# JiapengWu/TeMP

Measured on AMD Instinct MI355X. Metric: edges/sec (fwd+bwd) RGCN+GRU seq_len=15, higher is better.
Workload: dtype f32

## Files before the change

### temp_amd/csrc/gru_chain_hx.hpp

```cpp
#pragma once
#include "hx_pack.hpp"

namespace temp {

#define CHX_STATE_SCALE 16384.f
#define CHX_STATE_INV (1.f / 16384.f)

#define CHX_STAMP_EVENTS 8
#define CHX_STAMP_BLOCK (2 * CH_MAX_STEPS * CHX_STAMP_EVENTS)
#define CHX_STAMP_WORDS (2 * 2 * CHX_STAMP_BLOCK)
template <int DEV>
__device__ __forceinline__ long long* chx_stamp_rows(long long* stamp, int kernel, int role, bool first_wave, int lane) {
  if constexpr (DEV) {
    if (!stamp || !first_wave || lane != 0) return nullptr;
    const int mid = (int)(gridDim.x >> 1);
    const int sel = blockIdx.x == 0 ? 0 : ((int)blockIdx.x == mid ? 1 : -1);
    return sel < 0 ? nullptr : stamp + ((size_t)(kernel * 2 + sel) * 2 + role) * (CH_MAX_STEPS * CHX_STAMP_EVENTS);
  }
  return nullptr;
}
#define CHX_STAMP(s, k) do { if constexpr (DEV) { if (stp) stp[(s) * CHX_STAMP_EVENTS + (k)] = (long long)__builtin_readcyclecounter(); } } while (0)

struct ChainGeomHx {
  int NT, NS;
  int NTb, NSb;
  int lda, ldz;
  int ldp, ldpa;
  int ldh;
};
__host__ __device__ inline ChainGeomHx chain_geom_hx(int D) {
  ChainGeomHx g;
  g.NT = (3 * D + 31) >> 5; g.NS = (D + 15) >> 4;
  g.NTb = (D + 31) >> 5; g.NSb = (((3 * D + 15) >> 4) + 7) & ~7;
  g.lda = g.NT * 32 + 4; g.ldz = g.NTb * 32 + 4;
  g.ldp = g.NS * 32 + 16; g.ldpa = g.NSb * 32 + 16;
  g.ldh = g.NS * 16 + 4;
  return g;
}
inline size_t chain_lds_fwd_hx(int D, int ms) {
  const ChainGeomHx g = chain_geom_hx(D);
  return (size_t)CH_SLOTS * g.lda * 4 + 2 * (size_t)CH_SLOTS * g.ldp + (size_t)CH_SLOTS * g.ldh * 4 + (size_t)g.NT * 32 * 4 + (2 * CH_SLOTS + 1) * (size_t)ms * 4;
}
inline size_t chain_lds_bwd_hx(int D, int ms) {
  const ChainGeomHx g = chain_geom_hx(D);
  return 2 * (size_t)CH_SLOTS * g.ldpa + 2 * (size_t)CH_SLOTS * g.ldz * 4 + (2 * CH_SLOTS + 3) * (size_t)ms * 4 + CH_SLOTS * 4 + 4 * (size_t)D * 4;
}
inline size_t chain_hx_fwd_items(int D) { const ChainGeomHx g = chain_geom_hx(D); return (size_t)g.NS * g.NT * 128; }
inline size_t chain_hx_bwd_items(int D) { const ChainGeomHx g = chain_geom_hx(D); return (size_t)g.NSb * g.NTb * 128; }
inline size_t chain_hx_pack_floats(int D) {
  const ChainGeomHx g = chain_geom_hx(D);
  return (chain_hx_fwd_items(D) + chain_hx_bwd_items(D)) * 4 + (size_t)(g.NT + g.NTb) * 32;
}

template <int VARIANT, int TPW, int MW, int NMW = 4, int TWOSETS = 0>
__global__ void __launch_bounds__(64 * (NMW + MW)) k_gru_chain_fwd_hx(ChainArgs a, const float* __restrict__ gi, float* __restrict__ H,
                                                                       float* __restrict__ saved) {
  extern __shared__ __attribute__((aligned(16))) float lds[];
  constexpr int PASSES = CH_SLOTS / MW;
  const int D = a.D, D4 = D >> 2;
  const int G = (VARIANT == TEMP_GRU_TORCH) ? 3 * D : D;
  const ChainGeomHx g = chain_geom_hx(D);
  const int NT = g.NT, NS = g.NS, lda = g.lda, ldp = g.ldp, ldh = g.ldh;
  float* accb = lds;
  char* hpl = (char*)(accb + CH_SLOTS * lda);
  float* hb = (float*)(hpl + 2 * CH_SLOTS * ldp);
  float* ivt = hb + CH_SLOTS * ldh;
  int* tabb = (int*)(ivt + NT * 32);
  float* decb = (float*)(tabb + CH_SLOTS * a.max_steps);
  int* flagb = (int*)(decb + CH_SLOTS * a.max_steps);
  const int tid = threadIdx.x, wave = __builtin_amdgcn_readfirstlane(tid >> 6), lane = tid & 63;
  const size_t plane = a.plane;

  for (int p = blockIdx.x; p < a.n_panels; p += gridDim.x) {
    const int rnn_id = a.panel[4 * p], s0 = a.panel[4 * p + 1], ns = a.panel[4 * p + 2];
    const ChainRnn R = a.rnn[rnn_id];
    for (int i = tid; i < 2 * CH_SLOTS * ldp / 16; i += blockDim.x) reinterpret_cast<hx_u32x4*>(hpl)[i] = hx_u32x4{0u, 0u, 0u, 0u};
    for (int i = tid; i < CH_SLOTS * ldh; i += blockDim.x) hb[i] = 0.f;
    for (int i = tid; i < NT * 32; i += blockDim.x) ivt[i] = hx_inv_scale(R.kf[i]) * CHX_STATE_INV;
    for (int i = tid; i < ns * CH_SLOTS; i += blockDim.x) {
      const int e = a.rows[(size_t)s0 * CH_SLOTS + i];
      tabb[i] = e;
      decb[i] = e >= 0 ? decay_factor(a.dt[e & CH_ROW_MASK], a.lambda, R.decay_wb) : 0.f;
    }
    if (tid < ns) flagb[tid] = a.sinfo[4 * (size_t)(s0 + tid)];
    __syncthreads();

    if (wave < NMW) {
      const int li = lane & 31, hh = lane >> 5;
      bool tval[TPW];
      int tidx[TPW];
#pragma unroll
      for (int j = 0; j < TPW; ++j) { tidx[j] = wave + NMW * j; tval[j] = tidx[j] < NT; if (!tval[j]) tidx[j] = NT - 1; }
      f32x16 acc[TPW];
#pragma unroll
      for (int j = 0; j < TPW; ++j)
#pragma unroll
        for (int r = 0; r < 16; ++r) acc[j][r] = 0.f;
      const hx_u32x4* wp = reinterpret_cast<const hx_u32x4*>(R.wf);
      constexpr bool ONESET = NMW > 4 && !TWOSETS;
      constexpr bool PREF = !(NMW > 4 && TWOSETS);
      hx_u32x4 w[ONESET ? 1 : 2][2][TPW] = {};
      auto wload = [&](hx_u32x4 (&wr)[TPW], int sl, int pl) {
#pragma unroll
        for (int j = 0; j < TPW; ++j)
          if (tval[j]) wr[j] = wp[((size_t)(sl * NT + tidx[j]) * 2 + pl) * 64 + lane];
      };
      const int rot = (a.dbg & 64) ? 0 : (int)(blockIdx.x >> 3) % NS;
      wload(w[0][0], rot, 0); wload(w[0][1], rot, 1);
      if constexpr (!ONESET) { wload(w[1][0], rot + 1 < NS ? rot + 1 : 0, 0); wload(w[1][1], rot + 1 < NS ? rot + 1 : 0, 1); }
      const char* hrow = hpl + (size_t)li * ldp + 16 * hh;
      const int pl1 = CH_SLOTS * ldp;
      for (int s = 0; s < ns; ++s) {
        const int flags = flagb[s];
        if ((flags & 1) && !(a.dbg & 1)) {
          hx_u32x4 FH = *reinterpret_cast<const hx_u32x4*>(hrow + 32 * rot), FL = *reinterpret_cast<const hx_u32x4*>(hrow + pl1 + 32 * rot), NH, NL;
          int sl_cur = rot;
          auto slab = [&](auto set_c, int sl1, int sl2) {
            constexpr int SET = decltype(set_c)::value;
            if constexpr (PREF) {
              NH = *reinterpret_cast<const hx_u32x4*>(hrow + 32 * sl1);
              NL = *reinterpret_cast<const hx_u32x4*>(hrow + pl1 + 32 * sl1);
            } else {
              FH = *reinterpret_cast<const hx_u32x4*>(hrow + 32 * sl_cur);
              FL = *reinterpret_cast<const hx_u32x4*>(hrow + pl1 + 32 * sl_cur);
              sl_cur = sl1;
            }
            const hx_f16x8 ah = hx_frag(FH), al = hx_frag(FL);
            __builtin_amdgcn_sched_barrier(0);
#pragma unroll
            for (int j = 0; j < TPW; ++j) acc[j] = __builtin_amdgcn_mfma_f32_32x32x16_f16(hx_frag(w[SET][1][j]), ah, acc[j], 0, 0, 0);
            __builtin_amdgcn_sched_barrier(0);
            wload(w[SET][1], sl2, 1);
            __builtin_amdgcn_sched_barrier(0);
#pragma unroll
            for (int j = 0; j < TPW; ++j) acc[j] = __builtin_amdgcn_mfma_f32_32x32x16_f16(hx_frag(w[SET][0][j]), al, acc[j], 0, 0, 0);
#pragma unroll
            for (int j = 0; j < TPW; ++j) acc[j] = __builtin_amdgcn_mfma_f32_32x32x16_f16(hx_frag(w[SET][0][j]), ah, acc[j], 0, 0, 0);
            __builtin_amdgcn_sched_barrier(0);
            wload(w[SET][0], sl2, 0);
            if constexpr (PREF) { FH = NH; FL = NL; }
          };
          auto at = [&](int j) { const int v = rot + j; return v < NS ? v : v - NS; };
          if constexpr (ONESET) {
            for (int j = 0; j < NS; ++j) slab(std::integral_constant<int, 0>(), at(j + 1 < NS ? j + 1 : 0), at(j + 1 < NS ? j + 1 : 0));
          } else {
          int j = 0;
          for (; j + 1 < NS; j += 2) {
            slab(std::integral_constant<int, 0>(), at(j + 1), at(j + 2 < NS ? j + 2 : 0));
            slab(std::integral_constant<int, 1>(), at(j + 2 < NS ? j + 2 : 0), at(j + 3 < NS ? j + 3 : 1));
          }
          if (j < NS) slab(std::integral_constant<int, 0>(), at(0), at(0));
          }
#pragma unroll
          for (int j = 0; j < TPW; ++j) {
            if (!tval[j]) continue;
            float* dst = accb + (size_t)li * lda + tidx[j] * 32 + 4 * hh;
#pragma unroll
            for (int qq = 0; qq < 4; ++qq) {
              st4(dst + 8 * qq, make_float4(acc[j][4 * qq], acc[j][4 * qq + 1], acc[j][4 * qq + 2], acc[j][4 * qq + 3]));
              acc[j][4 * qq] = 0.f; acc[j][4 * qq + 1] = 0.f; acc[j][4 * qq + 2] = 0.f; acc[j][4 * qq + 3] = 0.f;
            }
          }
        }
        __syncthreads();
        __syncthreads();
      }
    } else {
      const int mw = wave - NMW, c4 = lane, col = 4 * c4;
      const bool cact = c4 < D4;
      const int colc = cact ? col : 0;
      const float4 bhr = ld4(R.b_hh + colc), bhz = ld4(R.b_hh + D + colc), bhn = ld4(R.b_hh + 2 * D + colc);
      int erow[PASSES];
      float4 g0[PASSES], g1[PASSES], g2[PASSES];
      auto prefetch = [&](int s) {
#pragma unroll
        for (int ps = 0; ps < PASSES; ++ps) {
          const int e = tabb[s * CH_SLOTS + ps * MW + mw];
          erow[ps] = e;
          const bool ok = e >= 0 && cact && !(a.dbg & 4);
          const int er = e & CH_ROW_MASK;
          const float* src = gi + (ok ? (size_t)(a.gi_index ? a.gi_index[er] : er) * G + col : 0);
          if (VARIANT == TEMP_GRU_TORCH) { g0[ps] = ld4(src); g1[ps] = ld4(src + (ok ? D : 0)); g2[ps] = ld4(src + (ok ? 2 * D : 0)); }
          else { g0[ps] = zero4(); g1[ps] = zero4(); g2[ps] = ld4(src); }
        }
      };
      prefetch(0);
      for (int s = 0; s < ns; ++s) {
        const int flags = flagb[s];
        __syncthreads();
#pragma unroll
        for (int ps = 0; ps < PASSES; ++ps) {
          const int slot = ps * MW + mw;
          const int e = erow[ps];
          if (e < 0 || !cact) continue;
          const size_t row = (size_t)(e & CH_ROW_MASK);
          const bool hp = (e & CH_HAS_PREV) != 0;
          float4 ar = zero4(), az = zero4(), an = zero4(), hd = zero4();
          if (hp) {
            const float* ab = accb + (size_t)slot * lda + col;
            const float dec = decb[s * CH_SLOTS + slot];
            const float4 pr = ld4(ab), pz = ld4(ab + D), pn = ld4(ab + 2 * D);
            const float4 ivr = ld4(ivt + col), ivz = ld4(ivt + D + col), ivn = ld4(ivt + 2 * D + col);
            ar = make_float4(pr.x * (ivr.x * dec), pr.y * (ivr.y * dec), pr.z * (ivr.z * dec), pr.w * (ivr.w * dec));
            az = make_float4(pz.x * (ivz.x * dec), pz.y * (ivz.y * dec), pz.z * (ivz.z * dec), pz.w * (ivz.w * dec));
            an = make_float4(pn.x * (ivn.x * dec), pn.y * (ivn.y * dec), pn.z * (ivn.z * dec), pn.w * (ivn.w * dec));
            hd = scale4(ld4(hb + (size_t)slot * ldh + col), dec);
          }
          float o_h[4], o_r[4], o_z[4], o_n[4], o_hn[4];
          const float arv[4] = {ar.x, ar.y, ar.z, ar.w}, azv[4] = {az.x, az.y, az.z, az.w}, anv[4] = {an.x, an.y, an.z, an.w};
          const float hdv[4] = {hd.x, hd.y, hd.z, hd.w};
          const float g0v[4] = {g0[ps].x, g0[ps].y, g0[ps].z, g0[ps].w}, g1v[4] = {g1[ps].x, g1[ps].y, g1[ps].z, g1[ps].w};
          const float g2v[4] = {g2[ps].x, g2[ps].y, g2[ps].z, g2[ps].w};
          const float brv[4] = {bhr.x, bhr.y, bhr.z, bhr.w}, bzv[4] = {bhz.x, bhz.y, bhz.z, bhz.w}, bnv[4] = {bhn.x, bhn.y, bhn.z, bhn.w};
#pragma unroll
          for (int k = 0; k < 4; ++k) {
            float xr = arv[k], xz = azv[k];
            if (VARIANT == TEMP_GRU_TORCH) { xr += g0v[k]; xz += g1v[k]; }
            const float rg = gate_sigmoid(xr + brv[k]);
            const float zg = gate_sigmoid(xz + bzv[k]);
            const float hn = anv[k] + bnv[k];
            const float ng = gate_tanh(g2v[k] + rg * hn);
            o_h[k] = (VARIANT == TEMP_GRU_TORCH) ? ((1.f - zg) * ng + zg * hdv[k]) : (ng + zg * (hdv[k] - ng));
            o_r[k] = rg; o_z[k] = zg; o_n[k] = ng; o_hn[k] = hn;
          }
          const float4 h4 = make_float4(o_h[0], o_h[1], o_h[2], o_h[3]);
          st4(hb + (size_t)slot * ldh + col, h4);
          hx_u32x2 SH, SL;
          hx_split4(h4, CHX_STATE_SCALE, SH, SL);
          char* hdst = hpl + (size_t)slot * ldp + 2 * col;
          *reinterpret_cast<hx_u32x2*>(hdst) = SH;
          *reinterpret_cast<hx_u32x2*>(hdst + CH_SLOTS * ldp) = SL;
          const size_t o = row * D + col;
          if (a.dbg & 2) continue;
          if (flags & 2) st4(H + o, h4);
          st4(saved + o, make_float4(o_r[0], o_r[1], o_r[2], o_r[3]));
          st4(saved + plane + o, make_float4(o_z[0], o_z[1], o_z[2], o_z[3]));
          st4(saved + 2 * plane + o, make_float4(o_n[0], o_n[1], o_n[2], o_n[3]));
          st4(saved + 3 * plane + o, make_float4(o_hn[0], o_hn[1], o_hn[2], o_hn[3]));
          st4(saved + 4 * plane + o, hd);
        }
        __syncthreads();
        if (s + 1 < ns) prefetch(s + 1);
      }
    }
    __syncthreads();
  }
}

struct ChainX {
  const float* x;
  const int32_t* x_index;
  const float* b_ih[TEMP_CHAIN_MAX_RNN];
  const hx_u32x4* wi[TEMP_CHAIN_MAX_RNN];
};
inline size_t chain_lds_fwd_x(int D, int ms) {
  const ChainGeomHx g = chain_geom_hx(D);
  return (size_t)CH_SLOTS * (3 * D + 4) * 4 + 4 * (size_t)CH_SLOTS * g.ldp + (size_t)CH_SLOTS * (D + 4) * 4 + CH_SLOTS * 4 + (2 * CH_SLOTS + 1) * (size_t)ms * 4;
}
template <int TPW, int MW, int NMW, int DEV = 0>
__global__ void __launch_bounds__(64 * (NMW + MW)) k_gru_chain_fwd_x(ChainArgs a, ChainX X, float* __restrict__ H, float* __restrict__ saved) {
  extern __shared__ __attribute__((aligned(16))) float lds[];
  constexpr int PASSES = CH_SLOTS / MW;
  const int D = a.D, D4 = D >> 2, G3 = 3 * D;
  const ChainGeomHx g = chain_geom_hx(D);
  const int NT = g.NT, NS = g.NS, ldp = g.ldp;
  const int lda = G3 + 4, ldn = D + 4;
  float* accb = lds;
  char* hpl = (char*)(accb + CH_SLOTS * lda);
  char* xpl = hpl + 2 * CH_SLOTS * ldp;
  float* gin = (float*)(xpl + 2 * CH_SLOTS * ldp);
  unsigned* xkey = (unsigned*)(gin + CH_SLOTS * ldn);
  int* tabb = (int*)(xkey + CH_SLOTS);
  float* decb = (float*)(tabb + CH_SLOTS * a.max_steps);
  int* flagb = (int*)(decb + CH_SLOTS * a.max_steps);
  const int tid = threadIdx.x, wave = __builtin_amdgcn_readfirstlane(tid >> 6), lane = tid & 63;
  const size_t plane = a.plane;
  const int dbg = DEV ? a.dbg : 0;

  if (wave < NMW) {
  for (int p = blockIdx.x; p < a.n_panels; p += gridDim.x) {
    const int rnn_id = a.panel[4 * p], s0 = a.panel[4 * p + 1], ns = a.panel[4 * p + 2];
    const ChainRnn R = a.rnn[rnn_id];
    for (int i = tid; i < 4 * CH_SLOTS * ldp / 16; i += blockDim.x) reinterpret_cast<hx_u32x4*>(hpl)[i] = hx_u32x4{0u, 0u, 0u, 0u};
    for (int i = tid; i < ns * CH_SLOTS; i += blockDim.x) {
      const int e = a.rows[(size_t)s0 * CH_SLOTS + i];
      tabb[i] = e;
      decb[i] = e >= 0 ? decay_factor(a.dt[e & CH_ROW_MASK], a.lambda, R.decay_wb) : 0.f;
    }
    if (tid < ns) flagb[tid] = a.sinfo[4 * (size_t)(s0 + tid)];
    __syncthreads();

      const int li = lane & 31, hh = lane >> 5;
      bool tval[TPW];
      int tidx[TPW];
#pragma unroll
      for (int j = 0; j < TPW; ++j) { tidx[j] = wave + NMW * j; tval[j] = tidx[j] < NT; if (!tval[j]) tidx[j] = NT - 1; }
      f32x16 acc[TPW];
#pragma unroll
      for (int j = 0; j < TPW; ++j)
#pragma unroll
        for (int r = 0; r < 16; ++r) acc[j][r] = 0.f;
      const hx_u32x4* wph = reinterpret_cast<const hx_u32x4*>(R.wf);
      const hx_u32x4* wpi = X.wi[rnn_id];
      hx_u32x4 w[2][TPW] = {};
      const std::integral_constant<int, 0> P0;
      const std::integral_constant<int, 1> P1;
      auto wload = [&](const hx_u32x4* wp, int sl, auto pl_c, int ln) __attribute__((always_inline)) {
        constexpr int pl = decltype(pl_c)::value;
#pragma unroll
        for (int j = 0; j < TPW; ++j)
          if (tval[j]) w[pl][j] = *reinterpret_cast<const hx_u32x4*>(reinterpret_cast<const char*>(wp) + (unsigned)((((sl * NT + tidx[j]) * 2 + pl) * 64 + ln) * 16));
      };
      const int rot = (dbg & 64) ? 0 : (int)(blockIdx.x >> 3) % NS;
      auto at = [&](int j) { const int v = rot + j; return v < NS ? v : v - NS; };
      const bool prio = !(dbg & 4096);
      bool holds_ih = true;
      wload(wpi, rot, P0, lane); wload(wpi, rot, P1, lane);
      auto walk = [&](const bool prod, const char* pl0, const hx_u32x4* wcur, const hx_u32x4* wnext) __attribute__((always_inline)) {
        int ln = lane;
        asm volatile("" : "+v"(ln));
        const char* arow = pl0 + (size_t)(ln & 31) * ldp + 16 * (ln >> 5);
        const int pl1 = CH_SLOTS * ldp;
        hx_u32x4 FH = *reinterpret_cast<const hx_u32x4*>(arow + 32 * rot), FL = *reinterpret_cast<const hx_u32x4*>(arow + pl1 + 32 * rot), NH, NL;
        if (prio) __builtin_amdgcn_s_setprio(2);
        for (int j = 0; j < NS; ++j) {
          const bool last = j + 1 == NS;
          const int sn = at(last ? 0 : j + 1);
          const hx_u32x4* wn = last ? wnext : wcur;
          NH = *reinterpret_cast<const hx_u32x4*>(arow + 32 * sn);
          NL = *reinterpret_cast<const hx_u32x4*>(arow + pl1 + 32 * sn);
          const hx_f16x8 ah = hx_frag(FH), al = hx_frag(FL);
          __builtin_amdgcn_sched_barrier(0);
#pragma unroll
          for (int t = 0; t < TPW; ++t) {
            if (prod) acc[t] = __builtin_amdgcn_mfma_f32_32x32x16_f16(hx_frag(w[1][t]), ah, acc[t], 0, 0, 0);
            else asm volatile("" : : "v"(w[1][t]));
          }
          __builtin_amdgcn_sched_barrier(0);
          wload(wn, sn, P1, ln);
          __builtin_amdgcn_sched_barrier(0);
          if (prod) {
#pragma unroll
            for (int t = 0; t < TPW; ++t) acc[t] = __builtin_amdgcn_mfma_f32_32x32x16_f16(hx_frag(w[0][t]), al, acc[t], 0, 0, 0);
#pragma unroll
            for (int t = 0; t < TPW; ++t) acc[t] = __builtin_amdgcn_mfma_f32_32x32x16_f16(hx_frag(w[0][t]), ah, acc[t], 0, 0, 0);
          } else {
#pragma unroll
            for (int t = 0; t < TPW; ++t) asm volatile("" : : "v"(w[0][t]));
          }
          __builtin_amdgcn_sched_barrier(0);
          wload(wn, sn, P0, ln);
          FH = NH; FL = NL;
        }
        if (prio) __builtin_amdgcn_s_setprio(0);
      };
      auto xprod = [&]() __attribute__((always_inline)) {
        if (!holds_ih) { wload(wpi, rot, P0, lane); wload(wpi, rot, P1, lane); }
        walk(!(dbg & (1 | 2048)), xpl, wpi, wph);
        holds_ih = false;
        const float f = hx_inv_scale(xkey[li]) * CHX_STATE_SCALE;
#pragma unroll
        for (int j = 0; j < TPW; ++j)
#pragma unroll
          for (int r = 0; r < 16; ++r) acc[j][r] *= f;
      };
      long long* stp = p == (int)blockIdx.x ? chx_stamp_rows<DEV>(a.stamp, 0, 0, wave == 0, lane) : nullptr;
      if (ns > 0) {
        __syncthreads();
        xprod();
        __syncthreads();
      }
      for (int s = 0; s < ns; ++s) {
        const int flags = flagb[s];
        CHX_STAMP(s, 0);
#pragma unroll
        for (int j = 0; j < TPW; ++j) {
          if (!tval[j]) continue;
#pragma unroll
          for (int qq = 0; qq < 4; ++qq) {
            const int c = tidx[j] * 32 + 8 * qq + 4 * hh;
            if (c < 2 * D || c >= G3) continue;
            st4(gin + (size_t)li * ldn + (c - 2 * D), make_float4(acc[j][4 * qq], acc[j][4 * qq + 1], acc[j][4 * qq + 2], acc[j][4 * qq + 3]));
            acc[j][4 * qq] = 0.f; acc[j][4 * qq + 1] = 0.f; acc[j][4 * qq + 2] = 0.f; acc[j][4 * qq + 3] = 0.f;
          }
        }
        if ((flags & 1) && !(dbg & 1)) {
          if (holds_ih) { wload(wph, rot, P0, lane); wload(wph, rot, P1, lane); }
          walk(true, hpl, wph, wpi);
          holds_ih = true;
        }
        CHX_STAMP(s, 1);
#pragma unroll
        for (int j = 0; j < TPW; ++j) {
          if (!tval[j]) continue;
          float* dst = accb + (size_t)li * lda + tidx[j] * 32 + 4 * hh;
#pragma unroll
          for (int qq = 0; qq < 4; ++qq) {
            if (tidx[j] * 32 + 8 * qq + 4 * hh < G3) st4(dst + 8 * qq, make_float4(acc[j][4 * qq], acc[j][4 * qq + 1], acc[j][4 * qq + 2], acc[j][4 * qq + 3]));
            acc[j][4 * qq] = 0.f; acc[j][4 * qq + 1] = 0.f; acc[j][4 * qq + 2] = 0.f; acc[j][4 * qq + 3] = 0.f;
          }
        }
        CHX_STAMP(s, 2);
        __syncthreads();
        CHX_STAMP(s, 3);
        if (s + 1 < ns) xprod();
        CHX_STAMP(s, 4);
        __syncthreads();
        CHX_STAMP(s, 5);
      }
    __syncthreads();
  }
  } else {
  for (int p = blockIdx.x; p < a.n_panels; p += gridDim.x) {
    const int rnn_id = a.panel[4 * p], s0 = a.panel[4 * p + 1], ns = a.panel[4 * p + 2];
    const ChainRnn R = a.rnn[rnn_id];
    for (int i = tid; i < 4 * CH_SLOTS * ldp / 16; i += blockDim.x) reinterpret_cast<hx_u32x4*>(hpl)[i] = hx_u32x4{0u, 0u, 0u, 0u};
    for (int i = tid; i < ns * CH_SLOTS; i += blockDim.x) {
      const int e = a.rows[(size_t)s0 * CH_SLOTS + i];
      tabb[i] = e;
      decb[i] = e >= 0 ? decay_factor(a.dt[e & CH_ROW_MASK], a.lambda, R.decay_wb) : 0.f;
    }
    if (tid < ns) flagb[tid] = a.sinfo[4 * (size_t)(s0 + tid)];
    __syncthreads();

      const int mw = wave - NMW, c4 = lane, col = 4 * c4;
      const bool cact = c4 < D4;
      const int colc = cact ? col : 0;
      const float* bih = X.b_ih[rnn_id];
      const float4 br = add4(ld4(bih + colc), ld4(R.b_hh + colc)), bz = add4(ld4(bih + D + colc), ld4(R.b_hh + D + colc));
      const float4 bhn = ld4(R.b_hh + 2 * D + colc), bin = ld4(bih + 2 * D + colc);
      float4 ivr, ivz, ivn;
      {
        const hx_u32x4 kr = *reinterpret_cast<const hx_u32x4*>(R.kf + colc), kz = *reinterpret_cast<const hx_u32x4*>(R.kf + D + colc);
        const hx_u32x4 kn = *reinterpret_cast<const hx_u32x4*>(R.kf + 2 * D + colc);
        auto iv = [](const hx_u32x4 k) { return make_float4(hx_inv_scale(k[0]) * CHX_STATE_INV, hx_inv_scale(k[1]) * CHX_STATE_INV,
                                                            hx_inv_scale(k[2]) * CHX_STATE_INV, hx_inv_scale(k[3]) * CHX_STATE_INV); };
        ivr = iv(kr); ivz = iv(kz); ivn = iv(kn);
      }
      float4 hdr[PASSES];
      float4 xr[PASSES];
      int xi[PASSES];
#pragma unroll
      for (int ps = 0; ps < PASSES; ++ps) hdr[ps] = zero4();
      typedef const int32_t __attribute__((address_space(4))) * chx_const_idx;
      const chx_const_idx xidx = (chx_const_idx)(uintptr_t)X.x_index;
      auto xindex = [&](int s) __attribute__((always_inline)) {
        int e[PASSES];
#pragma unroll
        for (int ps = 0; ps < PASSES; ++ps) e[ps] = tabb[s * CH_SLOTS + ps * MW + mw];
        __builtin_amdgcn_sched_barrier(0);
#pragma unroll
        for (int ps = 0; ps < PASSES; ++ps) {
          const int es = __builtin_amdgcn_readfirstlane(e[ps]);
          xi[ps] = (es >= 0 && !(dbg & 4)) ? xidx[es & CH_ROW_MASK] : -1;
        }
      };
      auto xload = [&]() __attribute__((always_inline)) {
#pragma unroll
        for (int ps = 0; ps < PASSES; ++ps) {
          xr[ps] = zero4();
          if (xi[ps] >= 0 && cact) xr[ps] = ld4(X.x + (size_t)xi[ps] * D + col);
        }
      };
      auto xsplit = [&]() __attribute__((always_inline)) {
#pragma unroll
        for (int ps = 0; ps < PASSES; ++ps) {
          const int slot = ps * MW + mw;
          const unsigned key = hx_wave_max(cact ? hx_abs_bits4(xr[ps]) : 0u);
          if (cact) {
            hx_u32x2 SH, SL;
            hx_split4(xr[ps], hx_scale(key), SH, SL);
            char* xd = xpl + (size_t)slot * ldp + 2 * col;
            *reinterpret_cast<hx_u32x2*>(xd) = SH;
            *reinterpret_cast<hx_u32x2*>(xd + CH_SLOTS * ldp) = SL;
          }
          if (lane == 0) xkey[slot] = key;
        }
      };
      long long* stp = p == (int)blockIdx.x ? chx_stamp_rows<DEV>(a.stamp, 0, 1, mw == 0, lane) : nullptr;
      if (ns > 0) {
        xindex(0);
        xload();
        if (ns > 1) xindex(1);
        xsplit();
        __syncthreads();
        if (ns > 1) xload();
        __syncthreads();
      }
      for (int s = 0; s < ns; ++s) {
        const int flags = flagb[s];
        CHX_STAMP(s, 0);
        if (s + 2 < ns) xindex(s + 2);
        if (s + 1 < ns) xsplit();
        CHX_STAMP(s, 1);
        __syncthreads();
        CHX_STAMP(s, 2);
        if (s + 2 < ns) xload();
        int colv = col;
        asm volatile("" : "+v"(colv));
        CHX_STAMP(s, 3);
#pragma unroll
        for (int ps = 0; ps < PASSES; ++ps) {
          const int slot = ps * MW + mw;
          const int e = tabb[s * CH_SLOTS + slot];
          if (!cact) continue;
          int en = -1;
          if (s + 1 < ns) en = tabb[(s + 1) * CH_SLOTS + slot];
          const bool hpn = en >= 0 && (en & CH_HAS_PREV);
          float4 h4 = zero4();
          if (e >= 0) {
            const size_t row = (size_t)(e & CH_ROW_MASK);
            const bool hp = (e & CH_HAS_PREV) != 0;
            const float* ab = accb + (size_t)slot * lda + colv;
            const float4 pr = ld4(ab), pz = ld4(ab + D), pn = ld4(ab + 2 * D), gn = ld4(gin + (size_t)slot * ldn + colv);
            const float4 hd = hp ? hdr[ps] : zero4();
            float o_h[4], o_r[4], o_z[4], o_n[4], o_hn[4];
            const float prv[4] = {pr.x, pr.y, pr.z, pr.w}, pzv[4] = {pz.x, pz.y, pz.z, pz.w}, pnv[4] = {pn.x, pn.y, pn.z, pn.w};
            const float ivrv[4] = {ivr.x, ivr.y, ivr.z, ivr.w}, ivzv[4] = {ivz.x, ivz.y, ivz.z, ivz.w}, ivnv[4] = {ivn.x, ivn.y, ivn.z, ivn.w};
            const float gnv[4] = {gn.x, gn.y, gn.z, gn.w}, hdv[4] = {hd.x, hd.y, hd.z, hd.w};
            const float brv[4] = {br.x, br.y, br.z, br.w}, bzv[4] = {bz.x, bz.y, bz.z, bz.w}, bnv[4] = {bhn.x, bhn.y, bhn.z, bhn.w};
            const float binv[4] = {bin.x, bin.y, bin.z, bin.w};
#pragma unroll
            for (int k = 0; k < 4; ++k) {
              const float rg = gate_sigmoid(prv[k] * ivrv[k] + brv[k]);
              const float zg = gate_sigmoid(pzv[k] * ivzv[k] + bzv[k]);
              const float hn = pnv[k] * ivnv[k] + bnv[k];
              const float ng = gate_tanh((gnv[k] * ivnv[k] + binv[k]) + rg * hn);
              o_h[k] = (1.f - zg) * ng + zg * hdv[k];
              o_r[k] = rg; o_z[k] = zg; o_n[k] = ng; o_hn[k] = hn;
            }
            h4 = make_float4(o_h[0], o_h[1], o_h[2], o_h[3]);
            const size_t o = row * D + col;
            if (!(a.dbg & 2)) {
              if (flags & 2) st4(H + o, h4);
              st4(saved + o, make_float4(o_r[0], o_r[1], o_r[2], o_r[3]));
              st4(saved + plane + o, make_float4(o_z[0], o_z[1], o_z[2], o_z[3]));
              st4(saved + 2 * plane + o, make_float4(o_n[0], o_n[1], o_n[2], o_n[3]));
              st4(saved + 3 * plane + o, make_float4(o_hn[0], o_hn[1], o_hn[2], o_hn[3]));
              st4(saved + 4 * plane + o, hd);
            }
          }
          if (s + 1 < ns) {
            hdr[ps] = hpn ? scale4(h4, decb[(s + 1) * CH_SLOTS + slot]) : zero4();
            hx_u32x2 SH, SL;
            hx_split4(hdr[ps], CHX_STATE_SCALE, SH, SL);
            char* hdst = hpl + (size_t)slot * ldp + 2 * colv;
            *reinterpret_cast<hx_u32x2*>(hdst) = SH;
            *reinterpret_cast<hx_u32x2*>(hdst + CH_SLOTS * ldp) = SL;
          }
        }
        CHX_STAMP(s, 4);
        __syncthreads();
        CHX_STAMP(s, 5);
      }
    __syncthreads();
  }
  }
}

template <int VARIANT, int TPWB, int MW, int G4, int NMW = 4, int RING = 4, int DEV = 0>
__global__ void __launch_bounds__(64 * (NMW + MW)) k_gru_chain_bwd_hx(ChainArgs a, ChainUps ups, const float* __restrict__ saved,
                                                                     float* __restrict__ dgi, float* __restrict__ dgh,
                                                                     unsigned* __restrict__ row_keys, unsigned* __restrict__ col_keys) {
  extern __shared__ __attribute__((aligned(16))) float lds[];
  constexpr int PASSES = CH_SLOTS / MW;
  const int D = a.D, D4 = D >> 2;
  const ChainGeomHx g = chain_geom_hx(D);
  const int NTb = g.NTb, NSb = g.NSb, ldpa = g.ldpa, ldz = g.ldz;
  char* apl = (char*)lds;
  float* gzb = (float*)(apl + 2 * CH_SLOTS * ldpa);
  float* dpb = gzb + CH_SLOTS * ldz;
  int* tabb = (int*)(dpb + CH_SLOTS * ldz);
  float* decb = (float*)(tabb + CH_SLOTS * a.max_steps);
  int* flagb = (int*)(decb + CH_SLOTS * a.max_steps);
  int* upb = flagb + a.max_steps;
  float* rinv = (float*)(upb + 2 * a.max_steps);
  unsigned* ckey = (unsigned*)(rinv + CH_SLOTS);
  const int tid = threadIdx.x, wave = __builtin_amdgcn_readfirstlane(tid >> 6), lane = tid & 63;
  const size_t plane = a.plane;

  for (int p = blockIdx.x; p < a.n_panels; p += gridDim.x) {
    const int rnn_id = a.panel[4 * p], s0 = a.panel[4 * p + 1], ns = a.panel[4 * p + 2];
    const ChainRnn R = a.rnn[rnn_id];
    for (int i = tid; i < 2 * CH_SLOTS * ldpa / 16; i += blockDim.x) reinterpret_cast<hx_u32x4*>(apl)[i] = hx_u32x4{0u, 0u, 0u, 0u};
    for (int i = tid; i < 4 * D; i += blockDim.x) ckey[i] = 0u;
    if (tid < ns) { upb[2 * tid] = a.sinfo[4 * (size_t)(s0 + tid) + 1]; upb[2 * tid + 1] = a.sinfo[4 * (size_t)(s0 + tid) + 2]; }
    for (int i = tid; i < ns * CH_SLOTS; i += blockDim.x) {
      const int e = a.rows[(size_t)s0 * CH_SLOTS + i];
      tabb[i] = e;
      decb[i] = e >= 0 ? decay_factor(a.dt[e & CH_ROW_MASK], a.lambda, R.decay_wb) : 0.f;
    }
    if (tid < ns) flagb[tid] = a.sinfo[4 * (size_t)(s0 + tid)];
    __syncthreads();

    if (wave < NMW) {
      const int li = lane & 31, hh = lane >> 5;
      bool tval[TPWB];
      int tidx[TPWB];
#pragma unroll
      for (int j = 0; j < TPWB; ++j) { tidx[j] = wave + NMW * j; tval[j] = tidx[j] < NTb; if (!tval[j]) tidx[j] = NTb - 1; }
      f32x16 acc[TPWB];
#pragma unroll
      for (int j = 0; j < TPWB; ++j)
#pragma unroll
        for (int r = 0; r < 16; ++r) acc[j][r] = 0.f;
      const hx_u32x4* wp = reinterpret_cast<const hx_u32x4*>(R.wb);
      hx_u32x4 wh[RING][TPWB] = {}, wl[RING][TPWB] = {};
      auto wload = [&](hx_u32x4 (&w)[TPWB], int sl, int pl) {
#pragma unroll
        for (int j = 0; j < TPWB; ++j)
          if (tval[j]) w[j] = wp[((size_t)(sl * NTb + tidx[j]) * 2 + pl) * 64 + lane];
      };
      const int rot = (a.dbg & 64) ? 0 : RING * ((int)(blockIdx.x >> 3) % (NSb / RING));
#pragma unroll
      for (int q = 0; q < RING; ++q) { wload(wh[q], rot + q, 0); wload(wl[q], rot + q, 1); }
      const char* arow = apl + (size_t)li * ldpa + 16 * hh;
      const int pl1 = CH_SLOTS * ldpa;
      long long* stp = p == (int)blockIdx.x ? chx_stamp_rows<DEV>(a.stamp, 1, 0, wave == 0, lane) : nullptr;
      for (int s = ns - 1; s >= 0; --s) {
        const int flags = flagb[s];
        CHX_STAMP(s, 0);
        __syncthreads();
        CHX_STAMP(s, 1);
        if ((flags & 1) && !(a.dbg & 1)) {
          hx_u32x4 FH = *reinterpret_cast<const hx_u32x4*>(arow + 32 * rot), FL = *reinterpret_cast<const hx_u32x4*>(arow + pl1 + 32 * rot), NH, NL;
          for (int j = 0, sl = rot; j < NSb; j += RING) {
            const int base2 = sl + RING < NSb ? sl + RING : 0;
#pragma unroll
            for (int q = 0; q < RING; ++q) {
              const int sn = (q < RING - 1) ? sl + q + 1 : base2;
              NH = *reinterpret_cast<const hx_u32x4*>(arow + 32 * sn);
              NL = *reinterpret_cast<const hx_u32x4*>(arow + pl1 + 32 * sn);
              const hx_f16x8 ah = hx_frag(FH), al = hx_frag(FL);
              __builtin_amdgcn_sched_barrier(0);
#pragma unroll
              for (int t = 0; t < TPWB; ++t) acc[t] = __builtin_amdgcn_mfma_f32_32x32x16_f16(hx_frag(wl[q][t]), ah, acc[t], 0, 0, 0);
              __builtin_amdgcn_sched_barrier(0);
              wload(wl[q], base2 + q, 1);
              __builtin_amdgcn_sched_barrier(0);
#pragma unroll
              for (int t = 0; t < TPWB; ++t) acc[t] = __builtin_amdgcn_mfma_f32_32x32x16_f16(hx_frag(wh[q][t]), al, acc[t], 0, 0, 0);
#pragma unroll
              for (int t = 0; t < TPWB; ++t) acc[t] = __builtin_amdgcn_mfma_f32_32x32x16_f16(hx_frag(wh[q][t]), ah, acc[t], 0, 0, 0);
              __builtin_amdgcn_sched_barrier(0);
              wload(wh[q], base2 + q, 0);
              FH = NH; FL = NL;
            }
            sl = base2;
          }
          CHX_STAMP(s, 2);
          const float dec = decb[s * CH_SLOTS + li], ri = rinv[li];
#pragma unroll
          for (int j = 0; j < TPWB; ++j) {
            if (!tval[j]) continue;
#pragma unroll
            for (int qq = 0; qq < 4; ++qq) {
              const int c = tidx[j] * 32 + 8 * qq + 4 * hh;
              const float4 gz = ld4(gzb + (size_t)li * ldz + c);
              const float i0 = hx_inv_scale(R.kb[c]) * ri, i1 = hx_inv_scale(R.kb[c + 1]) * ri, i2 = hx_inv_scale(R.kb[c + 2]) * ri, i3 = hx_inv_scale(R.kb[c + 3]) * ri;
              st4(dpb + (size_t)li * ldz + c, make_float4((acc[j][4 * qq] * i0 + gz.x) * dec, (acc[j][4 * qq + 1] * i1 + gz.y) * dec,
                                                           (acc[j][4 * qq + 2] * i2 + gz.z) * dec, (acc[j][4 * qq + 3] * i3 + gz.w) * dec));
              acc[j][4 * qq] = 0.f; acc[j][4 * qq + 1] = 0.f; acc[j][4 * qq + 2] = 0.f; acc[j][4 * qq + 3] = 0.f;
            }
          }
        }
        CHX_STAMP(s, 3);
        __syncthreads();
        CHX_STAMP(s, 4);
      }
    } else {
      const int mw = wave - NMW, c4 = lane, col = 4 * c4;
      const bool cact = c4 < D4;
      const int colc = cact ? col : 0;
      int erow[PASSES];
      int enx[PASSES];
      float4 sr[PASSES], sz[PASSES], sn[PASSES], shn[PASSES], shd[PASSES];
      unsigned ck[4][4] = {};
      auto prefetch = [&](int s) {
#pragma unroll
        for (int ps = 0; ps < PASSES; ++ps) {
          const int slot = ps * MW + mw;
          const int e = tabb[s * CH_SLOTS + slot];
          erow[ps] = e;
          int en = -1;
          if (s + 1 < ns) en = tabb[(s + 1) * CH_SLOTS + slot];
          enx[ps] = (en >= 0 && (en & CH_HAS_PREV)) ? en : -1;
          const bool ok = e >= 0 && cact && !(a.dbg & 4);
          const size_t row = ok ? (size_t)(e & CH_ROW_MASK) : 0;
          const float* src = saved + row * D + (ok ? col : 0);
          sr[ps] = ld4(src); sz[ps] = ld4(src + plane); sn[ps] = ld4(src + 2 * plane); shn[ps] = ld4(src + 3 * plane);
          shd[ps] = ld4(src + 4 * plane);
        }
      };
      long long* stp = p == (int)blockIdx.x ? chx_stamp_rows<DEV>(a.stamp, 1, 1, mw == 0, lane) : nullptr;
      prefetch(ns - 1);
      for (int s = ns - 1; s >= 0; --s) {
        CHX_STAMP(s, 0);
        const int up_sel = upb[2 * s], up_row0 = upb[2 * s + 1];
        const float* upp = up_sel >= 0 ? ups.p[up_sel] : nullptr;
#pragma unroll
        for (int ps = 0; ps < PASSES; ++ps) {
          const int slot = ps * MW + mw;
          const int e = erow[ps];
          if (e < 0) continue;
          const size_t row = (size_t)(e & CH_ROW_MASK);
          float4 gd = (upp && cact) ? ld4(upp + (row - (size_t)up_row0) * D + col) : zero4();
          if (enx[ps] >= 0 && cact) gd = add4(gd, ld4(dpb + (size_t)slot * ldz + col));
          const float4 rg = sr[ps], zg = sz[ps], ng = sn[ps], hn = shn[ps], hd = shd[ps];
          if (a.d_arg && enx[ps] >= 0) {
            const float part = cact ? chain_dot_prev(ld4(dpb + (size_t)slot * ldz + col), zg, ng, hd) : 0.f;
            chain_store_d_arg(a, R, enx[ps], part, lane);
          }
          float4 dr_pre, dz_pre, dn_pre, dhn, gz;
#define TEMP_GATE(c)                                          \
          {                                                   \
            const float dn = gd.c * (1.f - zg.c);             \
            const float dz = gd.c * (hd.c - ng.c);            \
            dn_pre.c = dn * (1.f - ng.c * ng.c);              \
            dr_pre.c = dn_pre.c * hn.c * rg.c * (1.f - rg.c); \
            dz_pre.c = dz * zg.c * (1.f - zg.c);              \
            dhn.c = dn_pre.c * rg.c;                          \
            gz.c = gd.c * zg.c;                               \
          }
          TEMP_GATE(x) TEMP_GATE(y) TEMP_GATE(z) TEMP_GATE(w)
#undef TEMP_GATE
          const unsigned kr = cact ? hx_abs_bits4(dr_pre) : 0u, kz = cact ? hx_abs_bits4(dz_pre) : 0u;
          const unsigned kn = cact ? hx_abs_bits4(dn_pre) : 0u, kh = cact ? hx_abs_bits4(dhn) : 0u;
          if (cact && col_keys) {
            if constexpr (NMW > 4) {
              auto upl = [&](int b4, const float4 v) {
                unsigned* k = ckey + b4 * D + col;
                atomicMax(k, hx_abs_bits(v.x)); atomicMax(k + 1, hx_abs_bits(v.y)); atomicMax(k + 2, hx_abs_bits(v.z)); atomicMax(k + 3, hx_abs_bits(v.w));
              };
              upl(0, dr_pre); upl(1, dz_pre); upl(2, dn_pre); upl(3, dhn);
            } else {
              auto upd = [](unsigned (&m)[4], const float4 v) { m[0] = max(m[0], hx_abs_bits(v.x)); m[1] = max(m[1], hx_abs_bits(v.y)); m[2] = max(m[2], hx_abs_bits(v.z)); m[3] = max(m[3], hx_abs_bits(v.w)); };
              upd(ck[0], dr_pre); upd(ck[1], dz_pre); upd(ck[2], dn_pre); upd(ck[3], dhn);
            }
          }
          const unsigned krz = max(kr, kz);
          const unsigned key_h = hx_wave_max(max(krz, kh));
          const float sc = hx_scale(key_h);
          if (cact) {
            hx_u32x2 SH, SL;
            char* ad = apl + (size_t)slot * ldpa + 2 * col;
            hx_split4(dr_pre, sc, SH, SL); *reinterpret_cast<hx_u32x2*>(ad) = SH; *reinterpret_cast<hx_u32x2*>(ad + CH_SLOTS * ldpa) = SL;
            hx_split4(dz_pre, sc, SH, SL); *reinterpret_cast<hx_u32x2*>(ad + 2 * D) = SH; *reinterpret_cast<hx_u32x2*>(ad + 2 * D + CH_SLOTS * ldpa) = SL;
            hx_split4(dhn, sc, SH, SL); *reinterpret_cast<hx_u32x2*>(ad + 4 * D) = SH; *reinterpret_cast<hx_u32x2*>(ad + 4 * D + CH_SLOTS * ldpa) = SL;
            st4(gzb + (size_t)slot * ldz + col, gz);
          }
          if (lane == 0) rinv[slot] = hx_inv_scale(key_h);
          if (row_keys) {
            const unsigned key_x = hx_wave_max(max(krz, kn));
            if (lane == 0) row_keys[row] = key_x;
          }
          if (cact && !(a.dbg & 2)) {
            if constexpr (G4) {
              const size_t b4 = row * 4 * D + col;
              st4(dgi + b4, dr_pre); st4(dgi + b4 + D, dz_pre); st4(dgi + b4 + 2 * D, dn_pre); st4(dgi + b4 + 3 * D, dhn);
            } else {
              const size_t b3 = row * 3 * D + col;
              if (VARIANT == TEMP_GRU_TORCH) { st4(dgi + b3, dr_pre); st4(dgi + b3 + D, dz_pre); st4(dgi + b3 + 2 * D, dn_pre); }
              else st4(dgi + row * D + col, dn_pre);
              st4(dgh + b3, dr_pre); st4(dgh + b3 + D, dz_pre); st4(dgh + b3 + 2 * D, dhn);
            }
          }
        }
        CHX_STAMP(s, 1);
        __syncthreads();
        CHX_STAMP(s, 2);
        if (s > 0) prefetch(s - 1);
        CHX_STAMP(s, 3);
        __syncthreads();
        CHX_STAMP(s, 4);
      }
      if (col_keys && cact && NMW <= 4) {
#pragma unroll
        for (int b4 = 0; b4 < 4; ++b4)
#pragma unroll
          for (int e = 0; e < 4; ++e) atomicMax(&ckey[b4 * D + colc + e], ck[b4][e]);
      }
    }
    __syncthreads();
    if (col_keys) {
      for (int i = tid; i < 4 * D; i += blockDim.x) col_keys[((size_t)a.n_rnn_keys + p) * 4 * D + i] = ckey[i];
      __syncthreads();
    }
  }
}

}
```

Measured before the change: 972.5 million.

## Specialize GRU chain tile count per wave and cache inverse key scales in LDS

The forward chain kernel now instantiates its per-wave tile loop with a compile-time count of valid tiles (TPW or TPW-1). This drops the per-tile validity predicates around weight loads, MFMAs and epilogue stores, and priming weight loads are ordered with scheduling barriers. The backward kernel skips the weight walk entirely for waves with no valid tile and removes predicates from its loads. It also precomputes the inverse key scales into a small LDS table once per panel instead of decoding them from global memory in the epilogue. The cost is a second inlined instantiation of the forward body, which may grow code size and register pressure, plus a little more LDS in the backward kernel.

```diff
diff --git a/temp_amd/csrc/gru_chain_hx.hpp b/temp_amd/csrc/gru_chain_hx.hpp
--- a/temp_amd/csrc/gru_chain_hx.hpp
+++ b/temp_amd/csrc/gru_chain_hx.hpp
@@ -43,7 +43,7 @@
 }
 inline size_t chain_lds_bwd_hx(int D, int ms) {
   const ChainGeomHx g = chain_geom_hx(D);
-  return 2 * (size_t)CH_SLOTS * g.ldpa + 2 * (size_t)CH_SLOTS * g.ldz * 4 + (2 * CH_SLOTS + 3) * (size_t)ms * 4 + CH_SLOTS * 4 + 4 * (size_t)D * 4;
+  return 2 * (size_t)CH_SLOTS * g.ldpa + 2 * (size_t)CH_SLOTS * g.ldz * 4 + (2 * CH_SLOTS + 3) * (size_t)ms * 4 + CH_SLOTS * 4 + 4 * (size_t)D * 4 + (size_t)g.NTb * 32 * 4;
 }
 inline size_t chain_hx_fwd_items(int D) { const ChainGeomHx g = chain_geom_hx(D); return (size_t)g.NS * g.NT * 128; }
 inline size_t chain_hx_bwd_items(int D) { const ChainGeomHx g = chain_geom_hx(D); return (size_t)g.NSb * g.NTb * 128; }
@@ -290,33 +290,44 @@
     if (tid < ns) flagb[tid] = a.sinfo[4 * (size_t)(s0 + tid)];
     __syncthreads();
 
+      auto role = [&](auto nv_c) __attribute__((always_inline)) {
+      constexpr int NV = decltype(nv_c)::value, NVA = NV > 0 ? NV : 1;
       const int li = lane & 31, hh = lane >> 5;
-      bool tval[TPW];
-      int tidx[TPW];
-#pragma unroll
-      for (int j = 0; j < TPW; ++j) { tidx[j] = wave + NMW * j; tval[j] = tidx[j] < NT; if (!tval[j]) tidx[j] = NT - 1; }
-      f32x16 acc[TPW];
-#pragma unroll
-      for (int j = 0; j < TPW; ++j)
+      int tidx[NVA];
+#pragma unroll
+      for (int j = 0; j < NVA; ++j) tidx[j] = wave + NMW * j < NT ? wave + NMW * j : NT - 1;
+      f32x16 acc[NVA];
+#pragma unroll
+      for (int j = 0; j < NVA; ++j)
 #pragma unroll
         for (int r = 0; r < 16; ++r) acc[j][r] = 0.f;
       const hx_u32x4* wph = reinterpret_cast<const hx_u32x4*>(R.wf);
       const hx_u32x4* wpi = X.wi[rnn_id];
-      hx_u32x4 w[2][TPW] = {};
+      hx_u32x4 w[2][NVA] = {};
       const std::integral_constant<int, 0> P0;
       const std::integral_constant<int, 1> P1;
       auto wload = [&](const hx_u32x4* wp, int sl, auto pl_c, int ln) __attribute__((always_inline)) {
         constexpr int pl = decltype(pl_c)::value;
 #pragma unroll
-        for (int j = 0; j < TPW; ++j)
-          if (tval[j]) w[pl][j] = *reinterpret_cast<const hx_u32x4*>(reinterpret_cast<const char*>(wp) + (unsigned)((((sl * NT + tidx[j]) * 2 + pl) * 64 + ln) * 16));
+        for (int j = 0; j < NV; ++j)
+          w[pl][j] = *reinterpret_cast<const hx_u32x4*>(reinterpret_cast<const char*>(wp) + (unsigned)((((sl * NT + tidx[j]) * 2 + pl) * 64 + ln) * 16));
       };
       const int rot = (dbg & 64) ? 0 : (int)(blockIdx.x >> 3) % NS;
       auto at = [&](int j) { const int v = rot + j; return v < NS ? v : v - NS; };
       const bool prio = !(dbg & 4096);
       bool holds_ih = true;
-      wload(wpi, rot, P0, lane); wload(wpi, rot, P1, lane);
+      auto prime = [&](const hx_u32x4* wp) __attribute__((always_inline)) {
+        int ln = lane;
+        asm volatile("" : "+v"(ln));
+        __builtin_amdgcn_sched_barrier(0);
+        wload(wp, rot, P1, ln);
+        __builtin_amdgcn_sched_barrier(0);
+        wload(wp, rot, P0, ln);
+        __builtin_amdgcn_sched_barrier(0);
+      };
+      prime(wpi);
       auto walk = [&](const bool prod, const char* pl0, const hx_u32x4* wcur, const hx_u32x4* wnext) __attribute__((always_inline)) {
+        if constexpr (NV == 0) return;
         int ln = lane;
         asm volatile("" : "+v"(ln));
         const char* arow = pl0 + (size_t)(ln & 31) * ldp + 16 * (ln >> 5);
@@ -332,7 +343,7 @@
           const hx_f16x8 ah = hx_frag(FH), al = hx_frag(FL);
           __builtin_amdgcn_sched_barrier(0);
 #pragma unroll
-          for (int t = 0; t < TPW; ++t) {
+          for (int t = 0; t < NV; ++t) {
             if (prod) acc[t] = __builtin_amdgcn_mfma_f32_32x32x16_f16(hx_frag(w[1][t]), ah, acc[t], 0, 0, 0);
             else asm volatile("" : : "v"(w[1][t]));
           }
@@ -341,12 +352,12 @@
           __builtin_amdgcn_sched_barrier(0);
           if (prod) {
 #pragma unroll
-            for (int t = 0; t < TPW; ++t) acc[t] = __builtin_amdgcn_mfma_f32_32x32x16_f16(hx_frag(w[0][t]), al, acc[t], 0, 0, 0);
-#pragma unroll
-            for (int t = 0; t < TPW; ++t) acc[t] = __builtin_amdgcn_mfma_f32_32x32x16_f16(hx_frag(w[0][t]), ah, acc[t], 0, 0, 0);
+            for (int t = 0; t < NV; ++t) acc[t] = __builtin_amdgcn_mfma_f32_32x32x16_f16(hx_frag(w[0][t]), al, acc[t], 0, 0, 0);
+#pragma unroll
+            for (int t = 0; t < NV; ++t) acc[t] = __builtin_amdgcn_mfma_f32_32x32x16_f16(hx_frag(w[0][t]), ah, acc[t], 0, 0, 0);
           } else {
 #pragma unroll
-            for (int t = 0; t < TPW; ++t) asm volatile("" : : "v"(w[0][t]));
+            for (int t = 0; t < NV; ++t) asm volatile("" : : "v"(w[0][t]));
           }
           __builtin_amdgcn_sched_barrier(0);
           wload(wn, sn, P0, ln);
@@ -355,12 +366,12 @@
         if (prio) __builtin_amdgcn_s_setprio(0);
       };
       auto xprod = [&]() __attribute__((always_inline)) {
-        if (!holds_ih) { wload(wpi, rot, P0, lane); wload(wpi, rot, P1, lane); }
+        if (!holds_ih) prime(wpi);
         walk(!(dbg & (1 | 2048)), xpl, wpi, wph);
         holds_ih = false;
         const float f = hx_inv_scale(xkey[li]) * CHX_STATE_SCALE;
 #pragma unroll
-        for (int j = 0; j < TPW; ++j)
+        for (int j = 0; j < NV; ++j)
 #pragma unroll
           for (int r = 0; r < 16; ++r) acc[j][r] *= f;
       };
@@ -374,8 +385,7 @@
         const int flags = flagb[s];
         CHX_STAMP(s, 0);
 #pragma unroll
-        for (int j = 0; j < TPW; ++j) {
-          if (!tval[j]) continue;
+        for (int j = 0; j < NV; ++j) {
 #pragma unroll
           for (int qq = 0; qq < 4; ++qq) {
             const int c = tidx[j] * 32 + 8 * qq + 4 * hh;
@@ -385,14 +395,13 @@
           }
         }
         if ((flags & 1) && !(dbg & 1)) {
-          if (holds_ih) { wload(wph, rot, P0, lane); wload(wph, rot, P1, lane); }
+          if (holds_ih) prime(wph);
           walk(true, hpl, wph, wpi);
           holds_ih = true;
         }
         CHX_STAMP(s, 1);
 #pragma unroll
-        for (int j = 0; j < TPW; ++j) {
-          if (!tval[j]) continue;
+        for (int j = 0; j < NV; ++j) {
           float* dst = accb + (size_t)li * lda + tidx[j] * 32 + 4 * hh;
 #pragma unroll
           for (int qq = 0; qq < 4; ++qq) {
@@ -408,6 +417,9 @@
         __syncthreads();
         CHX_STAMP(s, 5);
       }
+      };
+      if (wave + NMW * (TPW - 1) < NT) role(std::integral_constant<int, TPW>());
+      else role(std::integral_constant<int, TPW - 1>());
     __syncthreads();
   }
   } else {
@@ -570,7 +582,8 @@
   char* apl = (char*)lds;
   float* gzb = (float*)(apl + 2 * CH_SLOTS * ldpa);
   float* dpb = gzb + CH_SLOTS * ldz;
-  int* tabb = (int*)(dpb + CH_SLOTS * ldz);
+  float* kinv = dpb + CH_SLOTS * ldz;
+  int* tabb = (int*)(kinv + NTb * 32);
   float* decb = (float*)(tabb + CH_SLOTS * a.max_steps);
   int* flagb = (int*)(decb + CH_SLOTS * a.max_steps);
   int* upb = flagb + a.max_steps;
@@ -584,6 +597,7 @@
     const ChainRnn R = a.rnn[rnn_id];
     for (int i = tid; i < 2 * CH_SLOTS * ldpa / 16; i += blockDim.x) reinterpret_cast<hx_u32x4*>(apl)[i] = hx_u32x4{0u, 0u, 0u, 0u};
     for (int i = tid; i < 4 * D; i += blockDim.x) ckey[i] = 0u;
+    for (int i = tid; i < NTb * 32; i += blockDim.x) kinv[i] = hx_inv_scale(R.kb[i]);
     if (tid < ns) { upb[2 * tid] = a.sinfo[4 * (size_t)(s0 + tid) + 1]; upb[2 * tid + 1] = a.sinfo[4 * (size_t)(s0 + tid) + 2]; }
     for (int i = tid; i < ns * CH_SLOTS; i += blockDim.x) {
       const int e = a.rows[(size_t)s0 * CH_SLOTS + i];
@@ -594,7 +608,9 @@
     __syncthreads();
 
     if (wave < NMW) {
-      const int li = lane & 31, hh = lane >> 5;
+      int rl = lane;
+      asm volatile("" : "+v"(rl));
+      const int li = rl & 31, hh = rl >> 5;
       bool tval[TPWB];
       int tidx[TPWB];
 #pragma unroll
@@ -608,12 +624,19 @@
       hx_u32x4 wh[RING][TPWB] = {}, wl[RING][TPWB] = {};
       auto wload = [&](hx_u32x4 (&w)[TPWB], int sl, int pl) {
 #pragma unroll
-        for (int j = 0; j < TPWB; ++j)
-          if (tval[j]) w[j] = wp[((size_t)(sl * NTb + tidx[j]) * 2 + pl) * 64 + lane];
+        for (int j = 0; j < TPWB; ++j) w[j] = wp[((size_t)(sl * NTb + tidx[j]) * 2 + pl) * 64 + rl];
       };
       const int rot = (a.dbg & 64) ? 0 : RING * ((int)(blockIdx.x >> 3) % (NSb / RING));
-#pragma unroll
-      for (int q = 0; q < RING; ++q) { wload(wh[q], rot + q, 0); wload(wl[q], rot + q, 1); }
+      const bool walks = tval[0];
+      if (walks) {
+#pragma unroll
+        for (int q = 0; q < RING; ++q) {
+          wload(wl[q], rot + q, 1);
+          __builtin_amdgcn_sched_barrier(0);
+          wload(wh[q], rot + q, 0);
+          __builtin_amdgcn_sched_barrier(0);
+        }
+      }
       const char* arow = apl + (size_t)li * ldpa + 16 * hh;
       const int pl1 = CH_SLOTS * ldpa;
       long long* stp = p == (int)blockIdx.x ? chx_stamp_rows<DEV>(a.stamp, 1, 0, wave == 0, lane) : nullptr;
@@ -622,7 +645,7 @@
         CHX_STAMP(s, 0);
         __syncthreads();
         CHX_STAMP(s, 1);
-        if ((flags & 1) && !(a.dbg & 1)) {
+        if (walks && (flags & 1) && !(a.dbg & 1)) {
           hx_u32x4 FH = *reinterpret_cast<const hx_u32x4*>(arow + 32 * rot), FL = *reinterpret_cast<const hx_u32x4*>(arow + pl1 + 32 * rot), NH, NL;
           for (int j = 0, sl = rot; j < NSb; j += RING) {
             const int base2 = sl + RING < NSb ? sl + RING : 0;
@@ -657,7 +680,8 @@
             for (int qq = 0; qq < 4; ++qq) {
               const int c = tidx[j] * 32 + 8 * qq + 4 * hh;
               const float4 gz = ld4(gzb + (size_t)li * ldz + c);
-              const float i0 = hx_inv_scale(R.kb[c]) * ri, i1 = hx_inv_scale(R.kb[c + 1]) * ri, i2 = hx_inv_scale(R.kb[c + 2]) * ri, i3 = hx_inv_scale(R.kb[c + 3]) * ri;
+              const float4 kv = ld4(kinv + c);
+              const float i0 = kv.x * ri, i1 = kv.y * ri, i2 = kv.z * ri, i3 = kv.w * ri;
               st4(dpb + (size_t)li * ldz + c, make_float4((acc[j][4 * qq] * i0 + gz.x) * dec, (acc[j][4 * qq + 1] * i1 + gz.y) * dec,
                                                            (acc[j][4 * qq + 2] * i2 + gz.z) * dec, (acc[j][4 * qq + 3] * i3 + gz.w) * dec));
               acc[j][4 * qq] = 0.f; acc[j][4 * qq + 1] = 0.f; acc[j][4 * qq + 2] = 0.f; acc[j][4 * qq + 3] = 0.f;
```

Measured after the change: 988.2 million (median of 6 runs). +1.6%, better.
